# Jumpat/SegAnyGAussians

Hardware: AMD Instinct MI355X
Metric: train views/sec (fwd+bwd), 1080p, 1M Gaussians, 32-D features (higher is better)
Workload: dtype f32; 1 GPU; BASELINE cfg3: 1000000 Gaussians, 1920x1080, 32-D features, fwd+bwd, 1 view/GPU/step; parallelism=view-sharded x1

## Files before the change

### seganygaussians_amd/csrc/geometry.h

```cpp
#pragma once

#include "blend_rec.h"
#include "common.h"
#include "wave.h"

namespace mirast {

__device__ constexpr float SH_C0 = 0.28209479177387814f;
__device__ constexpr float SH_C1 = 0.4886025119029199f;
__device__ constexpr float SH_C2[5] = {1.0925484305920792f, -1.0925484305920792f, 0.31539156525252005f,
                                       -1.0925484305920792f, 0.5462742152960396f};
__device__ constexpr float SH_C3[7] = {-0.5900435899266435f, 2.890611442640554f, -0.4570457994644658f,
                                       0.3731763325901154f, -0.4570457994644658f, 1.445305721320277f,
                                       -0.5900435899266435f};

__device__ __forceinline__ void computeCov3D(const float3 scale, float mod, const float4 rot, float* cov3D)
{
    Mat3 S = {{{1.0f, 0, 0}, {0, 1.0f, 0}, {0, 0, 1.0f}}};
    S.m[0][0] = mod * scale.x;
    S.m[1][1] = mod * scale.y;
    S.m[2][2] = mod * scale.z;
    float r = rot.x, x = rot.y, y = rot.z, z = rot.w;
    Mat3 R = {{{1.f - 2.f * (y * y + z * z), 2.f * (x * y - r * z), 2.f * (x * z + r * y)},
               {2.f * (x * y + r * z), 1.f - 2.f * (x * x + z * z), 2.f * (y * z - r * x)},
// ... 311 lines not shown
    dL_dmean_acc.x += dm.x;
    dL_dmean_acc.y += dm.y;
    dL_dmean_acc.z += dm.z;
}

__device__ __forceinline__ void cov3d_backward(const float3 scale, float mod, const float4 rot, const float* dL_dcov3D,
                                               float3& dL_dscale, float4& dL_drot)
{
    const float r = rot.x, x = rot.y, y = rot.z, z = rot.w;
    const Mat3 R = {{{1.f - 2.f * (y * y + z * z), 2.f * (x * y - r * z), 2.f * (x * z + r * y)},
                     {2.f * (x * y + r * z), 1.f - 2.f * (x * x + z * z), 2.f * (y * z - r * x)},
                     {2.f * (x * z - r * y), 2.f * (y * z + r * x), 1.f - 2.f * (x * x + y * y)}}};
    Mat3 S = {{{1.0f, 0, 0}, {0, 1.0f, 0}, {0, 0, 1.0f}}};
    const float3 s = make_float3(mod * scale.x, mod * scale.y, mod * scale.z);
    S.m[0][0] = s.x;
    S.m[1][1] = s.y;
    S.m[2][2] = s.z;
    const Mat3 M = m3mul(S, R);
    const float* d = dL_dcov3D;
    const Mat3 dL_dSigma = {{{d[0], 0.5f * d[1], 0.5f * d[2]}, {0.5f * d[1], d[3], 0.5f * d[4]}, {0.5f * d[2], 0.5f * d[4], d[5]}}};
    Mat3 M2;
#pragma unroll
    for (int c = 0; c < 3; c++)
#pragma unroll
        for (int rr = 0; rr < 3; rr++) M2.m[c][rr] = 2.0f * M.m[c][rr];
    const Mat3 dL_dM = m3mul(M2, dL_dSigma);
    const Mat3 Rt = m3transpose(R);
    Mat3 dL_dMt = m3transpose(dL_dM);
    dL_dscale.x = Rt.m[0][0] * dL_dMt.m[0][0] + Rt.m[0][1] * dL_dMt.m[0][1] + Rt.m[0][2] * dL_dMt.m[0][2];
    dL_dscale.y = Rt.m[1][0] * dL_dMt.m[1][0] + Rt.m[1][1] * dL_dMt.m[1][1] + Rt.m[1][2] * dL_dMt.m[1][2];
    dL_dscale.z = Rt.m[2][0] * dL_dMt.m[2][0] + Rt.m[2][1] * dL_dMt.m[2][1] + Rt.m[2][2] * dL_dMt.m[2][2];
#pragma unroll
    for (int k = 0; k < 3; k++) {
        dL_dMt.m[0][k] *= s.x;
        dL_dMt.m[1][k] *= s.y;
        dL_dMt.m[2][k] *= s.z;
    }
    dL_drot.x = 2 * z * (dL_dMt.m[0][1] - dL_dMt.m[1][0]) + 2 * y * (dL_dMt.m[2][0] - dL_dMt.m[0][2]) + 2 * x * (dL_dMt.m[1][2] - dL_dMt.m[2][1]);
    dL_drot.y = 2 * y * (dL_dMt.m[1][0] + dL_dMt.m[0][1]) + 2 * z * (dL_dMt.m[2][0] + dL_dMt.m[0][2]) + 2 * r * (dL_dMt.m[1][2] - dL_dMt.m[2][1]) - 4 * x * (dL_dMt.m[2][2] + dL_dMt.m[1][1]);
    dL_drot.z = 2 * x * (dL_dMt.m[1][0] + dL_dMt.m[0][1]) + 2 * r * (dL_dMt.m[2][0] - dL_dMt.m[0][2]) + 2 * z * (dL_dMt.m[1][2] + dL_dMt.m[2][1]) - 4 * y * (dL_dMt.m[2][2] + dL_dMt.m[0][0]);
    dL_drot.w = 2 * r * (dL_dMt.m[0][1] - dL_dMt.m[1][0]) + 2 * x * (dL_dMt.m[2][0] + dL_dMt.m[0][2]) + 2 * y * (dL_dMt.m[1][2] + dL_dMt.m[2][1]) - 4 * z * (dL_dMt.m[1][1] + dL_dMt.m[0][0]);
}

__global__ void __launch_bounds__(256) geometry_bwd_kernel(
    int P, int D, int M, const float* __restrict__ means, const int* __restrict__ radii, const float* __restrict__ shs,
    const uint8_t* __restrict__ clamped, const float* __restrict__ scales, const float* __restrict__ rotations,
    const float* __restrict__ cov3Ds, ViewParams vp, const float* __restrict__ gpack ,
    float* __restrict__ dL_dmean2D, float* __restrict__ dL_dconics, float* __restrict__ dL_dopacity,
    float* __restrict__ dL_dmask, float* __restrict__ dL_dmeans, const float* __restrict__ dL_dcolor,
    float* __restrict__ dL_dcov, float* __restrict__ dL_dsh, float* __restrict__ dL_dscale, float* __restrict__ dL_drot)
{
    const int idx = blockIdx.x * blockDim.x + threadIdx.x;
    if (idx >= P) return;
    if (!(radii[idx] > 0)) {
        dL_dmean2D[3 * idx + 0] = dL_dmean2D[3 * idx + 1] = dL_dmean2D[3 * idx + 2] = 0.f;
        reinterpret_cast<float4*>(dL_dconics)[idx] = make_float4(0.f, 0.f, 0.f, 0.f);
        dL_dopacity[idx] = 0.f;
        if (dL_dmask) dL_dmask[idx] = 0.f;
#pragma unroll
        for (int i = 0; i < 6; i++) dL_dcov[(size_t)idx * 6 + i] = 0.f;
        dL_dmeans[3 * idx + 0] = dL_dmeans[3 * idx + 1] = dL_dmeans[3 * idx + 2] = 0.f;
        dL_dscale[3 * idx + 0] = dL_dscale[3 * idx + 1] = dL_dscale[3 * idx + 2] = 0.f;
        reinterpret_cast<float4*>(dL_drot)[idx] = make_float4(0.f, 0.f, 0.f, 0.f);
        return;
    }

    const float4 g0 = reinterpret_cast<const float4*>(gpack)[2 * idx];
    const float4 g1 = reinterpret_cast<const float4*>(gpack)[2 * idx + 1];
    dL_dmean2D[3 * idx + 0] = g0.x;
    dL_dmean2D[3 * idx + 1] = g0.y;
    dL_dmean2D[3 * idx + 2] = 0.f;
    reinterpret_cast<float4*>(dL_dconics)[idx] = make_float4(g0.z, g0.w, 0.f, g1.x);
    dL_dopacity[idx] = g1.y;
    if (dL_dmask) dL_dmask[idx] = g1.z;

    const float3 mean = make_float3(means[3 * idx], means[3 * idx + 1], means[3 * idx + 2]);
    const float3 dL_dconic = make_float3(g0.z, g0.w, g1.x);
    float cov3D[6];
#pragma unroll
    for (int i = 0; i < 6; i++) cov3D[i] = cov3Ds[(size_t)idx * 6 + i];
    Cov2DCtx c;
    cov2d_common(mean, vp, cov3D, c);
    const float h_x = vp.focal_x, h_y = vp.focal_y;
    const float limx = 1.3f * vp.tan_fovx;
    const float limy = 1.3f * vp.tan_fovy;
    const float x_grad_mul = c.txtz < -limx || c.txtz > limx ? 0 : 1;
    const float y_grad_mul = c.tytz < -limy || c.tytz > limy ? 0 : 1;
    const Mat3& T = c.T;
    const Mat3& Vrk = c.Vrk;
    const Mat3& Wm = c.W;
    const float3 t = c.t;
    const float a = c.cov.m[0][0];
    const float b = c.cov.m[0][1];
    const float cc = c.cov.m[1][1];
    const float denom = a * cc - b * b;
    float dL_da = 0, dL_db = 0, dL_dc = 0;
    const float denom2inv = 1.0f / ((denom * denom) + 0.0000001f);
    float dcov[6];
    if (denom2inv != 0) {
        dL_da = denom2inv * (-cc * cc * dL_dconic.x + 2 * b * cc * dL_dconic.y + (denom - a * cc) * dL_dconic.z);
        dL_dc = denom2inv * (-a * a * dL_dconic.z + 2 * a * b * dL_dconic.y + (denom - a * cc) * dL_dconic.x);
        dL_db = denom2inv * 2 * (b * cc * dL_dconic.x - (denom + 2 * b * b) * dL_dconic.y + a * b * dL_dconic.z);
        dcov[0] = (T.m[0][0] * T.m[0][0] * dL_da + T.m[0][0] * T.m[1][0] * dL_db + T.m[1][0] * T.m[1][0] * dL_dc);
        dcov[3] = (T.m[0][1] * T.m[0][1] * dL_da + T.m[0][1] * T.m[1][1] * dL_db + T.m[1][1] * T.m[1][1] * dL_dc);
        dcov[5] = (T.m[0][2] * T.m[0][2] * dL_da + T.m[0][2] * T.m[1][2] * dL_db + T.m[1][2] * T.m[1][2] * dL_dc);
        dcov[1] = 2 * T.m[0][0] * T.m[0][1] * dL_da + (T.m[0][0] * T.m[1][1] + T.m[0][1] * T.m[1][0]) * dL_db + 2 * T.m[1][0] * T.m[1][1] * dL_dc;
        dcov[2] = 2 * T.m[0][0] * T.m[0][2] * dL_da + (T.m[0][0] * T.m[1][2] + T.m[0][2] * T.m[1][0]) * dL_db + 2 * T.m[1][0] * T.m[1][2] * dL_dc;
        dcov[4] = 2 * T.m[0][2] * T.m[0][1] * dL_da + (T.m[0][1] * T.m[1][2] + T.m[0][2] * T.m[1][1]) * dL_db + 2 * T.m[1][1] * T.m[1][2] * dL_dc;
    } else {
#pragma unroll
        for (int i = 0; i < 6; i++) dcov[i] = 0;
    }
#pragma unroll
    for (int i = 0; i < 6; i++) dL_dcov[(size_t)idx * 6 + i] = dcov[i];

    const float dL_dT00 = 2 * (T.m[0][0] * Vrk.m[0][0] + T.m[0][1] * Vrk.m[0][1] + T.m[0][2] * Vrk.m[0][2]) * dL_da +
                          (T.m[1][0] * Vrk.m[0][0] + T.m[1][1] * Vrk.m[0][1] + T.m[1][2] * Vrk.m[0][2]) * dL_db;
    const float dL_dT01 = 2 * (T.m[0][0] * Vrk.m[1][0] + T.m[0][1] * Vrk.m[1][1] + T.m[0][2] * Vrk.m[1][2]) * dL_da +
                          (T.m[1][0] * Vrk.m[1][0] + T.m[1][1] * Vrk.m[1][1] + T.m[1][2] * Vrk.m[1][2]) * dL_db;
    const float dL_dT02 = 2 * (T.m[0][0] * Vrk.m[2][0] + T.m[0][1] * Vrk.m[2][1] + T.m[0][2] * Vrk.m[2][2]) * dL_da +
                          (T.m[1][0] * Vrk.m[2][0] + T.m[1][1] * Vrk.m[2][1] + T.m[1][2] * Vrk.m[2][2]) * dL_db;
    const float dL_dT10 = 2 * (T.m[1][0] * Vrk.m[0][0] + T.m[1][1] * Vrk.m[0][1] + T.m[1][2] * Vrk.m[0][2]) * dL_dc +
                          (T.m[0][0] * Vrk.m[0][0] + T.m[0][1] * Vrk.m[0][1] + T.m[0][2] * Vrk.m[0][2]) * dL_db;
    const float dL_dT11 = 2 * (T.m[1][0] * Vrk.m[1][0] + T.m[1][1] * Vrk.m[1][1] + T.m[1][2] * Vrk.m[1][2]) * dL_dc +
                          (T.m[0][0] * Vrk.m[1][0] + T.m[0][1] * Vrk.m[1][1] + T.m[0][2] * Vrk.m[1][2]) * dL_db;
    const float dL_dT12 = 2 * (T.m[1][0] * Vrk.m[2][0] + T.m[1][1] * Vrk.m[2][1] + T.m[1][2] * Vrk.m[2][2]) * dL_dc +
                          (T.m[0][0] * Vrk.m[2][0] + T.m[0][1] * Vrk.m[2][1] + T.m[0][2] * Vrk.m[2][2]) * dL_db;
    const float dL_dJ00 = Wm.m[0][0] * dL_dT00 + Wm.m[0][1] * dL_dT01 + Wm.m[0][2] * dL_dT02;
    const float dL_dJ02 = Wm.m[2][0] * dL_dT00 + Wm.m[2][1] * dL_dT01 + Wm.m[2][2] * dL_dT02;
    const float dL_dJ11 = Wm.m[1][0] * dL_dT10 + Wm.m[1][1] * dL_dT11 + Wm.m[1][2] * dL_dT12;
    const float dL_dJ12 = Wm.m[2][0] * dL_dT10 + Wm.m[2][1] * dL_dT11 + Wm.m[2][2] * dL_dT12;
    const float tz = 1.f / t.z;
    const float tz2 = tz * tz;
    const float tz3 = tz2 * tz;
    const float dL_dtx = x_grad_mul * -h_x * tz2 * dL_dJ02;
    const float dL_dty = y_grad_mul * -h_y * tz2 * dL_dJ12;
    const float dL_dtz = -h_x * tz2 * dL_dJ00 - h_y * tz2 * dL_dJ11 + (2 * h_x * t.x) * tz3 * dL_dJ02 + (2 * h_y * t.y) * tz3 * dL_dJ12;
    float3 dL_dmean_acc = transformVec4x3Transpose(make_float3(dL_dtx, dL_dty, dL_dtz), vp.view);

    const float* proj = vp.proj;
    const float4 m_hom = transformPoint4x4(mean, proj);
    const float m_w = 1.0f / (m_hom.w + 0.0000001f);
    const float mul1 = (proj[0] * mean.x + proj[4] * mean.y + proj[8] * mean.z + proj[12]) * m_w * m_w;
    const float mul2 = (proj[1] * mean.x + proj[5] * mean.y + proj[9] * mean.z + proj[13]) * m_w * m_w;
    const float gx = g0.x, gy = g0.y;
    float3 dm;
    dm.x = (proj[0] * m_w - proj[3] * mul1) * gx + (proj[1] * m_w - proj[3] * mul2) * gy;
    dm.y = (proj[4] * m_w - proj[7] * mul1) * gx + (proj[5] * m_w - proj[7] * mul2) * gy;
    dm.z = (proj[8] * m_w - proj[11] * mul1) * gx + (proj[9] * m_w - proj[11] * mul2) * gy;
    dL_dmean_acc.x += dm.x;
    dL_dmean_acc.y += dm.y;
    dL_dmean_acc.z += dm.z;
    if (shs) sh_backward(idx, D, M, mean, vp, shs, clamped, dL_dcolor, dL_dmean_acc, dL_dsh);
    dL_dmeans[3 * idx + 0] = dL_dmean_acc.x;
    dL_dmeans[3 * idx + 1] = dL_dmean_acc.y;
    dL_dmeans[3 * idx + 2] = dL_dmean_acc.z;
    if (scales) {
        const float3 s = make_float3(scales[3 * idx], scales[3 * idx + 1], scales[3 * idx + 2]);
        const float4 q = reinterpret_cast<const float4*>(rotations)[idx];
        float3 ds;
        float4 dq;
        cov3d_backward(s, vp.scale_modifier, q, dcov, ds, dq);
        dL_dscale[3 * idx + 0] = ds.x;
        dL_dscale[3 * idx + 1] = ds.y;
        dL_dscale[3 * idx + 2] = ds.z;
        reinterpret_cast<float4*>(dL_drot)[idx] = dq;
    } else {
        dL_dscale[3 * idx + 0] = dL_dscale[3 * idx + 1] = dL_dscale[3 * idx + 2] = 0.f;
        reinterpret_cast<float4*>(dL_drot)[idx] = make_float4(0.f, 0.f, 0.f, 0.f);
    }
}

__global__ void __launch_bounds__(256) unpack_mask_kernel(int P, const float* __restrict__ gpack, float* __restrict__ dL_dmask)
{
    const int idx = blockIdx.x * blockDim.x + threadIdx.x;
    if (idx < P) dL_dmask[idx] = gpack[(size_t)idx * 8 + 6];
}

}
```

### seganygaussians_amd/csrc/mi_rast.hip

```cpp
#include "host.h"

#include <algorithm>
#include <atomic>
#include <cstdio>
#include <cstdlib>
#include <cstring>
#include <mutex>
#include <type_traits>
#include <utility>
#include <vector>

#include "bin_full.h"
#include "bin_lean.h"
#include "tile_ranges.h"
#include "tile_sort.h"
#include "blend_bwd.h"
#include "blend_bwd_wave.h"
#include "blend_bwd_feat.h"
#include "blend_fwd.h"
#include "blend_fwd_wave.h"
#ifdef MI_RAST_PROFILING
#include "blend_fwd_x3.h"
#endif
#include "common.h"
// ... 406 lines not shown
                });
            }
        } else {
            hipLaunchKernelGGL(bin_spans_kernel<true>, dim3(bp.nwg), dim3(1024), span_lds_bytes((size_t)bp.lean_band_h * c.vp.grid_x), c.stream,
                               P, c.geom.index_rec, c.geom.depth_key, c.geom.band_bits, c.img.tile_count, c.img.tile_cursor, c.img.ranges, c.bin.entries,
                               c.vp.grid_x, c.vp.grid_y, bp.lean_band_h, bp.lean_nbands, (const int*)c.img.num_rendered, (int*)nullptr);
        }
    }
    STAGE_CHECK(c, "emit entries");
    if (verify) {
        uint32_t* ctr = reinterpret_cast<uint32_t*>(c.img.words() + NR_VERIFY);
        HIP_TRY(hipMemsetAsync(ctr, 0, sizeof(uint32_t), c.stream));
        hipLaunchKernelGGL(verify_entries_kernel, dim3(ntiles), dim3(256), 0, c.stream, (uint32_t)ntiles, c.img.ranges, c.bin.entries, ctr);
        uint32_t unwritten = 0;
        HIP_TRY(hipMemcpyAsync(&unwritten, ctr, sizeof(uint32_t), hipMemcpyDeviceToHost, c.stream));
        HIP_TRY(hipStreamSynchronize(c.stream));
        if (unwritten)
            return fail(MI_RAST_ERR_HIP, "internal error: " + std::to_string(unwritten) + " list slots were counted but not emitted "
                                         "(count / emit passes of bin_spans_kernel disagree)");
    }
    return MI_RAST_OK;
}

int take_longest_run(Call& c, const HostSync& hs, int dev)
{
    HIP_TRY(hipEventSynchronize(hs.ev2));
    c.longest_run = longest_of(hs.words() + NR_RUN_BOUNDS, c.ntiles());
    g_last_longest_run[dev] = (int)c.longest_run;
    return MI_RAST_OK;
}

template <int CLASS>
void launch_tile_sort_wave(const Call& c)
{
    hipLaunchKernelGGL(tile_sort_wave_kernel<CLASS>, dim3((c.ntiles() + 3) / 4), dim3(256), 0, c.stream, c.ntiles(), c.img.ranges,
                       (const uint2*)c.bin.entries, c.bin.blend_list);
}
template <int LO, int CAP, bool FB, int NT>
void launch_tile_sort(const Call& c)
{
    hipLaunchKernelGGL((tile_sort_kernel<LO, CAP, FB, NT>), dim3(c.ntiles()), dim3(NT), 0, c.stream, c.ntiles(), c.img.ranges, c.bin.entries,
                       c.bin.scratch, (const int*)(c.img.words() + NR_KEY_BITS), c.bin.blend_list);
}

int sort_stage(Call& c, const BinPlan& bp, const HostSync& hs, int dev, int R)
{
    {
        StageTimer t(c.stream, MI_STAGE_TILE_SORT);
        launch_tile_sort_wave<0>(c);
        if (int rc = take_longest_run(c, hs, dev)) return rc;
        if (bp.full ? hs.words()[NR_TOTAL] != R : hs.words()[NR_TOTAL] > R)
            return fail(MI_RAST_ERR_HIP, "internal error: tile counts do not add up to num_rendered");
        const int max_tile_count = hs.words()[NR_LONGEST];
        if (max_tile_count > 1024) launch_tile_sort_wave<1>(c);
        if (max_tile_count > 2048) launch_tile_sort_wave<2>(c);
        if (max_tile_count > TILE_SORT_WAVE_MAX) launch_tile_sort<TILE_SORT_WAVE_MAX, 6144, false, 1024>(c);
        if (max_tile_count > 6144) launch_tile_sort<6144, 8192, true, 1024>(c);
    }
    STAGE_CHECK(c, "tile sort");
    return MI_RAST_OK;
}

int geometry_and_binning(Call& c, const FrontArgs& a, int* num_rendered)
{
    const int dev = current_device();
    if (dev < 0) return fail(MI_RAST_ERR_HIP, "hipGetDevice failed (or device ordinal >= 64)");
    HostSync& hs = g_host_sync_tl[dev];
    BinPlan bp;
    if (int rc = plan_binning(c, bp)) return rc;
    size_t goff[MI_GEOM_NFIELDS], ioff[MI_IMG_NFIELDS], boff[MI_BIN_NFIELDS];
    char* geom_base = a.geometry_buffer(mi_rast_geometry_layout(c.P, goff), a.geometry_user);
    if (!geom_base) return fail(MI_RAST_ERR_ALLOC, "geometry buffer callback returned NULL");
    c.geom = geom_from(geom_base, c.P);
    char* img_base = a.image_buffer(mi_rast_image_layout(c.vp.W, c.vp.H, ioff), a.image_user);
    if (!img_base) return fail(MI_RAST_ERR_ALLOC, "image buffer callback returned NULL");
    c.img = img_from(img_base, c.vp.W, c.vp.H);

    if (int rc = preprocess_stage(c, a, bp)) return rc;
    if (int rc = opt_in_to_large_lds(dev)) return rc;
    if (!hs.init()) return fail(MI_RAST_ERR_HIP, "cannot allocate pinned host buffer / event");
    if (int rc = count_and_scan_stage(c, bp, hs)) return rc;
    HIP_TRY(hipEventRecord(hs.ev2, c.stream));
    HIP_TRY(hipEventSynchronize(hs.ev));
    long long Rsum = 0;
    for (int k = 0; k < R_SLOTS; k++) Rsum += hs.pinned[k * R_SLOT_STRIDE];
    if (Rsum > 0x7fffffffll) return fail(MI_RAST_ERR_INVALID, "more than 2^31 tile overlaps");
    const int R = (int)Rsum;
    *num_rendered = R;

    char* bin_base = a.binning_buffer(mi_rast_binning_layout(R, boff), a.binning_user);
    if (!bin_base) return fail(MI_RAST_ERR_ALLOC, "binning buffer callback returned NULL");
    c.bin = bin_from(bin_base, R);
    if (R == 0) return take_longest_run(c, hs, dev);
    if (int rc = emit_stage(c, bp, R)) return rc;
    return sort_stage(c, bp, hs, dev, R);
}

struct FwdArgs { int channels; const float *features, *mask, *bg; float *out_color, *out_mask, *out_depth; };
struct BwdArgs { int channels; const float *bg, *colors, *dL_dpix, *dL_dout_mask; float* dL_dcolor; };

template <int C, int EXTRA>
void launch_blend_fwd(const Call& c, const FwdArgs& a, ChannelBlock b)
{
    constexpr bool MAY_BE_PARTIAL = C == 16 && EXTRA == 0;
    with_bools(MAY_BE_PARTIAL && b.real < C, c.xexp(), [&](auto partial, auto xexp) {
        if constexpr (MAY_BE_PARTIAL || !decltype(partial)::value)
            hipLaunchKernelGGL((blend_fwd_kernel<C, EXTRA, decltype(xexp)::value, decltype(partial)::value>), dim3(c.vp.grid_x, c.vp.grid_y), dim3(256), 0,
                               c.stream, c.img.ranges, c.bin.blend_list, c.geom.index_rec, c.vp.W, c.vp.H, a.features + b.c0, a.mask, c.geom.depths,
// ... 522 lines not shown
```

### seganygaussians_amd/csrc/tile_sort.h

```cpp
#pragma once

#include "blend_rec.h"
#include "wave.h"

namespace mirast {

struct LdsPairs {
    uint32_t* k;
    uint32_t* v;
    __device__ __forceinline__ uint32_t key(int i) const { return k[i]; }
    __device__ __forceinline__ uint32_t val(int i) const { return v[i]; }
    __device__ __forceinline__ void set(int i, uint32_t kk, uint32_t vv) const
    {
        k[i] = kk;
        v[i] = vv;
    }
};
struct GlobalPairs {
    uint2* p;
    __device__ __forceinline__ uint32_t key(int i) const { return p[i].x; }
    __device__ __forceinline__ uint32_t val(int i) const { return p[i].y; }
    __device__ __forceinline__ void set(int i, uint32_t kk, uint32_t vv) const { p[i] = make_uint2(kk, vv); }
};

template <int NW, int MAXB, typename Src, typename Dst>
__device__ __forceinline__ void radix_pass(Src src, Dst dst, int n, int shift, uint32_t (*s_hist)[256], int tid)
{
    const int lane = tid & 63, wave = tid >> 6;
    const int chunks = (n + 63) >> 6;
    const int cpw = (chunks + NW - 1) / NW;
    const int begin = min(n, wave * cpw * 64), end = min(n, (wave + 1) * cpw * 64);
    for (int d = tid; d < NW * 256; d += NW * 64) (&s_hist[0][0])[d] = 0;
    __syncthreads();

    auto match = [&](uint32_t digit, bool active, uint32_t& rank_in_wave, uint32_t& cnt) {
        uint64_t m = ballot64(active);
#pragma unroll
        for (int b = 0; b < 8; b++) {
            const uint64_t bal = ballot64(active && ((digit >> b) & 1u));
            m &= ((digit >> b) & 1u) ? bal : ~bal;
        }
        rank_in_wave = __builtin_amdgcn_mbcnt_hi((uint32_t)(m >> 32), __builtin_amdgcn_mbcnt_lo((uint32_t)m, 0u));
        cnt = (uint32_t)__builtin_popcountll(m);
    };

    constexpr int NB = MAXB > 0 ? MAXB : 1;
    uint32_t c_key[NB], c_val[NB], c_rk[NB], c_cnt[NB];
    if (MAXB > 0) {
#pragma unroll
        for (int j = 0; j < NB; j++) {
            const int i0 = begin + 64 * j;
            if (i0 >= end) break;
            const int i = i0 + lane;
            const bool active = i < end;
            c_key[j] = active ? src.key(i) : 0u;
// ... 57 lines not shown
        for (int i0 = begin; i0 < end; i0 += 64) {
            const int i = i0 + lane;
            const bool active = i < end;
            const uint32_t key = active ? src.key(i) : 0u, val = active ? src.val(i) : 0u;
            uint32_t rk, cnt;
            match((key >> shift) & 0xFFu, active, rk, cnt);
            scatter(key, val, active, rk, cnt);
        }
    }
    __syncthreads();
}

template <int NW, typename Src>
__device__ __forceinline__ void emit_blend_list(Src sorted, int n, uint2 range, int tid, uint32_t* __restrict__ blend_list)
{
    uint32_t* out = blend_list + range.x;
    for (int i = tid; i < n; i += NW * 64) {
        const uint32_t k = sorted.key(i), v = sorted.val(i);
        int pos = i;
        if ((i > 0 && sorted.key(i - 1) == k) || (i + 1 < n && sorted.key(i + 1) == k)) {
            int lo = i, hi = i + 1;
            while (lo > 0 && sorted.key(lo - 1) == k) lo--;
            while (hi < n && sorted.key(hi) == k) hi++;
            int before = 0;
            for (int q = lo; q < hi; q++) before += (sorted.val(q) & ID_MASK) < (v & ID_MASK) ? 1 : 0;
            pos = lo + before;
        }
        out[pos] = v;
    }
}

__global__ void __launch_bounds__(256) verify_entries_kernel(uint32_t ntiles, const uint2* __restrict__ ranges,
                                                              const uint2* __restrict__ entries, uint32_t* __restrict__ unwritten)
{
    const uint32_t tile = blockIdx.x;
    if (tile >= ntiles) return;
    const uint2 r = ranges[tile];
    uint32_t n = 0;
    for (uint32_t i = r.x + threadIdx.x; i < r.y; i += 256) n += entries[i].y == 0u;
    if (n) atomicAdd(unwritten, n);
}

__device__ __forceinline__ void minmax64(double& lo, double& hi)
{
    double mn;
    asm("v_min_f64 %0, %1, %2" : "=v"(mn) : "v"(lo), "v"(hi));
    asm("v_max_f64 %0, %1, %2" : "=v"(hi) : "v"(lo), "v"(hi));
    lo = mn;
}

template <int EPL, int K, int J, bool FLIP>
__device__ __forceinline__ void bitonic_step(double (&a)[EPL], int lane)
{
    if constexpr (FLIP && K > EPL) {
        constexpr int M = K / EPL - 1;
        const bool lower = (lane & ((M + 1) >> 1)) == 0;
#pragma unroll
        for (int r = 0; r < EPL / 2; r++) {
            double x0 = a[r], y0 = lane_xor64<M>(a[EPL - 1 - r]);
            double x1 = a[EPL - 1 - r], y1 = lane_xor64<M>(a[r]);
            minmax64(x0, y0);
            minmax64(x1, y1);
            a[r] = lower ? x0 : y0;
            a[EPL - 1 - r] = lower ? x1 : y1;
        }
    } else if constexpr (!FLIP && J >= EPL) {
        constexpr int M = J / EPL;
        const bool lower = (lane & M) == 0;
#pragma unroll
        for (int r = 0; r < EPL; r++) {
            double x = a[r], y = lane_xor64<M>(a[r]);
            minmax64(x, y);
            a[r] = lower ? x : y;
        }
    } else {
        constexpr int X = FLIP ? K - 1 : J;
#pragma unroll
        for (int r = 0; r < EPL; r++)
            if ((r ^ X) > r) minmax64(a[r], a[r ^ X]);
    }
}
template <int EPL, int K, int J>
__device__ __forceinline__ void bitonic_tail(double (&a)[EPL], int lane)
{
    if constexpr (J >= 1) {
        bitonic_step<EPL, K, J, false>(a, lane);
        bitonic_tail<EPL, K, J / 2>(a, lane);
    } else if constexpr (K < 64 * EPL) {
        bitonic_step<EPL, 2 * K, 0, true>(a, lane);
        bitonic_tail<EPL, 2 * K, K / 2>(a, lane);
    }
}

template <int EPL>
__device__ __forceinline__ void tile_sort_in_wave(const uint2* __restrict__ seg, int n, uint32_t* __restrict__ out, int lane)
{
    double a[EPL];
#pragma unroll
    for (int r = 0; r < EPL; r++) {
        const int e = r * 64 + lane;
        uint64_t w = 0x7FEFFFFFFFFFFFFFull;
        if (e < n) {
            const uint2 p = seg[e];
            w = ((uint64_t)p.x << 32) | __builtin_rotateleft32(p.y, 4);
        }
        a[r] = __builtin_bit_cast(double, w);
    }
    bitonic_step<EPL, 2, 0, true>(a, lane);
    bitonic_tail<EPL, 2, 0>(a, lane);
#pragma unroll
    for (int r = 0; r < EPL; r++) {
        const int e = lane * EPL + r;
        if (e < n) out[e] = __builtin_rotateright32((uint32_t)__builtin_bit_cast(uint64_t, a[r]), 4);
    }
}

constexpr int TILE_SORT_WAVE_MAX = 4096;
template <int CLASS>
__global__ void __launch_bounds__(256) tile_sort_wave_kernel(uint32_t ntiles, const uint2* __restrict__ ranges,
                                                              const uint2* __restrict__ entries, uint32_t* __restrict__ blend_list)
{
    const int lane = threadIdx.x & 63;
    const uint32_t tile = blockIdx.x * 4u + (threadIdx.x >> 6);
    if (tile >= ntiles) return;
    const uint2 range = ranges[tile];
    const int n = (int)(range.y - range.x);
    const uint2* seg = entries + range.x;
    uint32_t* out = blend_list + range.x;
    if constexpr (CLASS == 2) {
        if (n > 2048 && n <= 4096) tile_sort_in_wave<64>(seg, n, out, lane);
    } else if constexpr (CLASS == 1) {
        if (n > 1024 && n <= 2048) tile_sort_in_wave<32>(seg, n, out, lane);
    } else {
        if (n == 0 || n > 1024) return;
        if (n <= 256) tile_sort_in_wave<4>(seg, n, out, lane);
        else if (n <= 512) tile_sort_in_wave<8>(seg, n, out, lane);
        else tile_sort_in_wave<16>(seg, n, out, lane);
    }
}

template <int LO, int CAP, bool GLOBAL_FALLBACK, int NT>
__global__ void __launch_bounds__(NT) tile_sort_kernel(uint32_t ntiles, const uint2* __restrict__ ranges,
                                                        uint2* __restrict__ entries, uint2* __restrict__ scratch,
                                                        const int* __restrict__ key_bits, uint32_t* __restrict__ blend_list)
{
    __shared__ uint32_t s_k[2][CAP];
    __shared__ uint32_t s_v[2][CAP];
    constexpr int NW = NT / 64;
    __shared__ uint32_t s_hist[NW][256];
    const int tid = threadIdx.x;
    const uint32_t tile = blockIdx.x;
    if (tile >= ntiles) return;
    const uint2 range = ranges[tile];
    const int passes = (*key_bits + 7) >> 3;
    const int n = (int)(range.y - range.x);
    if (n <= LO) return;
    if (n > CAP && !GLOBAL_FALLBACK) return;
    uint2* seg = entries + range.x;
    if (n <= CAP) {
        for (int i = tid; i < n; i += NT) {
            const uint2 e = seg[i];
            s_k[0][i] = e.x;
            s_v[0][i] = e.y;
        }
        __syncthreads();
        int cur = 0;
        for (int p = 0; p < passes; p++, cur ^= 1)
            radix_pass<NW, (CAP + NW * 64 - 1) / (NW * 64)>(LdsPairs{s_k[cur], s_v[cur]}, LdsPairs{s_k[cur ^ 1], s_v[cur ^ 1]}, n, 8 * p, s_hist, tid);
        emit_blend_list<NW>(LdsPairs{s_k[cur], s_v[cur]}, n, range, tid, blend_list);
    } else {
        uint2* a = seg;
        uint2* b = scratch + range.x;
        for (int p = 0; p < passes; p++) {
            radix_pass<NW, 0>(GlobalPairs{a}, GlobalPairs{b}, n, 8 * p, s_hist, tid);
            uint2* t = a;
            a = b;
            b = t;
        }
        emit_blend_list<NW>(GlobalPairs{a}, n, range, tid, blend_list);
    }
}

}
```

Measured before the change: 910.5 views/s.

## Add 3/4-size in-wave sort classes and skip zero-gradient rows in geometry backward

Adds an in-lane sorting network that handles element-per-lane counts of 6, 12, 24 and 48, and splits the tile-sort size classes so tiles of 257-384, 513-768, 1025-1536 and 2049-3072 entries are padded less. It also restructures the geometry backward kernel to skip the full gradient computation when all packed 2D gradients are zero and no SH or mask gradients are needed, writing zeros from a single store path. The new sorting network and extra kernel launch add code complexity and a compile-time risk for non-power-of-two bitonic correctness.

Result: no change. 914.9 views/s, median of 6 (+0.5%).

```diff
diff --git a/seganygaussians_amd/csrc/geometry.h b/seganygaussians_amd/csrc/geometry.h
--- a/seganygaussians_amd/csrc/geometry.h
+++ b/seganygaussians_amd/csrc/geometry.h
@@ -387,123 +387,113 @@
 {
     const int idx = blockIdx.x * blockDim.x + threadIdx.x;
     if (idx >= P) return;
-    if (!(radii[idx] > 0)) {
-        dL_dmean2D[3 * idx + 0] = dL_dmean2D[3 * idx + 1] = dL_dmean2D[3 * idx + 2] = 0.f;
-        reinterpret_cast<float4*>(dL_dconics)[idx] = make_float4(0.f, 0.f, 0.f, 0.f);
-        dL_dopacity[idx] = 0.f;
-        if (dL_dmask) dL_dmask[idx] = 0.f;
-#pragma unroll
-        for (int i = 0; i < 6; i++) dL_dcov[(size_t)idx * 6 + i] = 0.f;
-        dL_dmeans[3 * idx + 0] = dL_dmeans[3 * idx + 1] = dL_dmeans[3 * idx + 2] = 0.f;
-        dL_dscale[3 * idx + 0] = dL_dscale[3 * idx + 1] = dL_dscale[3 * idx + 2] = 0.f;
-        reinterpret_cast<float4*>(dL_drot)[idx] = make_float4(0.f, 0.f, 0.f, 0.f);
-        return;
-    }
-
-    const float4 g0 = reinterpret_cast<const float4*>(gpack)[2 * idx];
-    const float4 g1 = reinterpret_cast<const float4*>(gpack)[2 * idx + 1];
+    bool zero_row = !(radii[idx] > 0);
+    float4 g0 = make_float4(0.f, 0.f, 0.f, 0.f), g1 = g0;
+    if (!zero_row) {
+        g0 = reinterpret_cast<const float4*>(gpack)[2 * idx];
+        g1 = reinterpret_cast<const float4*>(gpack)[2 * idx + 1];
+        zero_row = shs == nullptr && dL_dmask == nullptr && g0.x == 0.f && g0.y == 0.f && g0.z == 0.f && g0.w == 0.f && g1.x == 0.f &&
+                   g1.y == 0.f;
+    }
+    float dcov[6] = {0.f, 0.f, 0.f, 0.f, 0.f, 0.f};
+    float3 dmean = make_float3(0.f, 0.f, 0.f), ds = make_float3(0.f, 0.f, 0.f);
+    float4 dq = make_float4(0.f, 0.f, 0.f, 0.f);
+    if (!zero_row) {
+        const float3 mean = make_float3(means[3 * idx], means[3 * idx + 1], means[3 * idx + 2]);
+        const float3 dL_dconic = make_float3(g0.z, g0.w, g1.x);
+        float cov3D[6];
+#pragma unroll
+        for (int i = 0; i < 6; i++) cov3D[i] = cov3Ds[(size_t)idx * 6 + i];
+        Cov2DCtx c;
+        cov2d_common(mean, vp, cov3D, c);
+        const float h_x = vp.focal_x, h_y = vp.focal_y;
+        const float limx = 1.3f * vp.tan_fovx;
+        const float limy = 1.3f * vp.tan_fovy;
+        const float x_grad_mul = c.txtz < -limx || c.txtz > limx ? 0 : 1;
+        const float y_grad_mul = c.tytz < -limy || c.tytz > limy ? 0 : 1;
+        const Mat3& T = c.T;
+        const Mat3& Vrk = c.Vrk;
+        const Mat3& Wm = c.W;
+        const float3 t = c.t;
+        const float a = c.cov.m[0][0];
+        const float b = c.cov.m[0][1];
+        const float cc = c.cov.m[1][1];
+        const float denom = a * cc - b * b;
+        float dL_da = 0, dL_db = 0, dL_dc = 0;
+        const float denom2inv = 1.0f / ((denom * denom) + 0.0000001f);
+        if (denom2inv != 0) {
+            dL_da = denom2inv * (-cc * cc * dL_dconic.x + 2 * b * cc * dL_dconic.y + (denom - a * cc) * dL_dconic.z);
+            dL_dc = denom2inv * (-a * a * dL_dconic.z + 2 * a * b * dL_dconic.y + (denom - a * cc) * dL_dconic.x);
+            dL_db = denom2inv * 2 * (b * cc * dL_dconic.x - (denom + 2 * b * b) * dL_dconic.y + a * b * dL_dconic.z);
+            dcov[0] = (T.m[0][0] * T.m[0][0] * dL_da + T.m[0][0] * T.m[1][0] * dL_db + T.m[1][0] * T.m[1][0] * dL_dc);
+            dcov[3] = (T.m[0][1] * T.m[0][1] * dL_da + T.m[0][1] * T.m[1][1] * dL_db + T.m[1][1] * T.m[1][1] * dL_dc);
+            dcov[5] = (T.m[0][2] * T.m[0][2] * dL_da + T.m[0][2] * T.m[1][2] * dL_db + T.m[1][2] * T.m[1][2] * dL_dc);
+            dcov[1] = 2 * T.m[0][0] * T.m[0][1] * dL_da + (T.m[0][0] * T.m[1][1] + T.m[0][1] * T.m[1][0]) * dL_db + 2 * T.m[1][0] * T.m[1][1] * dL_dc;
+            dcov[2] = 2 * T.m[0][0] * T.m[0][2] * dL_da + (T.m[0][0] * T.m[1][2] + T.m[0][2] * T.m[1][0]) * dL_db + 2 * T.m[1][0] * T.m[1][2] * dL_dc;
+            dcov[4] = 2 * T.m[0][2] * T.m[0][1] * dL_da + (T.m[0][1] * T.m[1][2] + T.m[0][2] * T.m[1][1]) * dL_db + 2 * T.m[1][1] * T.m[1][2] * dL_dc;
+        }
+
+        const float dL_dT00 = 2 * (T.m[0][0] * Vrk.m[0][0] + T.m[0][1] * Vrk.m[0][1] + T.m[0][2] * Vrk.m[0][2]) * dL_da +
+                              (T.m[1][0] * Vrk.m[0][0] + T.m[1][1] * Vrk.m[0][1] + T.m[1][2] * Vrk.m[0][2]) * dL_db;
+        const float dL_dT01 = 2 * (T.m[0][0] * Vrk.m[1][0] + T.m[0][1] * Vrk.m[1][1] + T.m[0][2] * Vrk.m[1][2]) * dL_da +
+                              (T.m[1][0] * Vrk.m[1][0] + T.m[1][1] * Vrk.m[1][1] + T.m[1][2] * Vrk.m[1][2]) * dL_db;
+        const float dL_dT02 = 2 * (T.m[0][0] * Vrk.m[2][0] + T.m[0][1] * Vrk.m[2][1] + T.m[0][2] * Vrk.m[2][2]) * dL_da +
+                              (T.m[1][0] * Vrk.m[2][0] + T.m[1][1] * Vrk.m[2][1] + T.m[1][2] * Vrk.m[2][2]) * dL_db;
+        const float dL_dT10 = 2 * (T.m[1][0] * Vrk.m[0][0] + T.m[1][1] * Vrk.m[0][1] + T.m[1][2] * Vrk.m[0][2]) * dL_dc +
+                              (T.m[0][0] * Vrk.m[0][0] + T.m[0][1] * Vrk.m[0][1] + T.m[0][2] * Vrk.m[0][2]) * dL_db;
+        const float dL_dT11 = 2 * (T.m[1][0] * Vrk.m[1][0] + T.m[1][1] * Vrk.m[1][1] + T.m[1][2] * Vrk.m[1][2]) * dL_dc +
+                              (T.m[0][0] * Vrk.m[1][0] + T.m[0][1] * Vrk.m[1][1] + T.m[0][2] * Vrk.m[1][2]) * dL_db;
+        const float dL_dT12 = 2 * (T.m[1][0] * Vrk.m[2][0] + T.m[1][1] * Vrk.m[2][1] + T.m[1][2] * Vrk.m[2][2]) * dL_dc +
+                              (T.m[0][0] * Vrk.m[2][0] + T.m[0][1] * Vrk.m[2][1] + T.m[0][2] * Vrk.m[2][2]) * dL_db;
+        const float dL_dJ00 = Wm.m[0][0] * dL_dT00 + Wm.m[0][1] * dL_dT01 + Wm.m[0][2] * dL_dT02;
+        const float dL_dJ02 = Wm.m[2][0] * dL_dT00 + Wm.m[2][1] * dL_dT01 + Wm.m[2][2] * dL_dT02;
+        const float dL_dJ11 = Wm.m[1][0] * dL_dT10 + Wm.m[1][1] * dL_dT11 + Wm.m[1][2] * dL_dT12;
+        const float dL_dJ12 = Wm.m[2][0] * dL_dT10 + Wm.m[2][1] * dL_dT11 + Wm.m[2][2] * dL_dT12;
+        const float tz = 1.f / t.z;
+        const float tz2 = tz * tz;
+        const float tz3 = tz2 * tz;
+        const float dL_dtx = x_grad_mul * -h_x * tz2 * dL_dJ02;
+        const float dL_dty = y_grad_mul * -h_y * tz2 * dL_dJ12;
+        const float dL_dtz = -h_x * tz2 * dL_dJ00 - h_y * tz2 * dL_dJ11 + (2 * h_x * t.x) * tz3 * dL_dJ02 + (2 * h_y * t.y) * tz3 * dL_dJ12;
+        float3 dL_dmean_acc = transformVec4x3Transpose(make_float3(dL_dtx, dL_dty, dL_dtz), vp.view);
+
+        const float* proj = vp.proj;
+        const float4 m_hom = transformPoint4x4(mean, proj);
+        const float m_w = 1.0f / (m_hom.w + 0.0000001f);
+        const float mul1 = (proj[0] * mean.x + proj[4] * mean.y + proj[8] * mean.z + proj[12]) * m_w * m_w;
+        const float mul2 = (proj[1] * mean.x + proj[5] * mean.y + proj[9] * mean.z + proj[13]) * m_w * m_w;
+        const float gx = g0.x, gy = g0.y;
+        float3 dm;
+        dm.x = (proj[0] * m_w - proj[3] * mul1) * gx + (proj[1] * m_w - proj[3] * mul2) * gy;
+        dm.y = (proj[4] * m_w - proj[7] * mul1) * gx + (proj[5] * m_w - proj[7] * mul2) * gy;
+        dm.z = (proj[8] * m_w - proj[11] * mul1) * gx + (proj[9] * m_w - proj[11] * mul2) * gy;
+        dL_dmean_acc.x += dm.x;
+        dL_dmean_acc.y += dm.y;
+        dL_dmean_acc.z += dm.z;
+        if (shs) sh_backward(idx, D, M, mean, vp, shs, clamped, dL_dcolor, dL_dmean_acc, dL_dsh);
+        dmean = dL_dmean_acc;
+        if (scales) {
+            const float3 s = make_float3(scales[3 * idx], scales[3 * idx + 1], scales[3 * idx + 2]);
+            const float4 q = reinterpret_cast<const float4*>(rotations)[idx];
+            cov3d_backward(s, vp.scale_modifier, q, dcov, ds, dq);
+        }
+    }
+
     dL_dmean2D[3 * idx + 0] = g0.x;
     dL_dmean2D[3 * idx + 1] = g0.y;
     dL_dmean2D[3 * idx + 2] = 0.f;
     reinterpret_cast<float4*>(dL_dconics)[idx] = make_float4(g0.z, g0.w, 0.f, g1.x);
     dL_dopacity[idx] = g1.y;
     if (dL_dmask) dL_dmask[idx] = g1.z;
-
-    const float3 mean = make_float3(means[3 * idx], means[3 * idx + 1], means[3 * idx + 2]);
-    const float3 dL_dconic = make_float3(g0.z, g0.w, g1.x);
-    float cov3D[6];
-#pragma unroll
-    for (int i = 0; i < 6; i++) cov3D[i] = cov3Ds[(size_t)idx * 6 + i];
-    Cov2DCtx c;
-    cov2d_common(mean, vp, cov3D, c);
-    const float h_x = vp.focal_x, h_y = vp.focal_y;
-    const float limx = 1.3f * vp.tan_fovx;
-    const float limy = 1.3f * vp.tan_fovy;
-    const float x_grad_mul = c.txtz < -limx || c.txtz > limx ? 0 : 1;
-    const float y_grad_mul = c.tytz < -limy || c.tytz > limy ? 0 : 1;
-    const Mat3& T = c.T;
-    const Mat3& Vrk = c.Vrk;
-    const Mat3& Wm = c.W;
-    const float3 t = c.t;
-    const float a = c.cov.m[0][0];
-    const float b = c.cov.m[0][1];
-    const float cc = c.cov.m[1][1];
-    const float denom = a * cc - b * b;
-    float dL_da = 0, dL_db = 0, dL_dc = 0;
-    const float denom2inv = 1.0f / ((denom * denom) + 0.0000001f);
-    float dcov[6];
-    if (denom2inv != 0) {
-        dL_da = denom2inv * (-cc * cc * dL_dconic.x + 2 * b * cc * dL_dconic.y + (denom - a * cc) * dL_dconic.z);
-        dL_dc = denom2inv * (-a * a * dL_dconic.z + 2 * a * b * dL_dconic.y + (denom - a * cc) * dL_dconic.x);
-        dL_db = denom2inv * 2 * (b * cc * dL_dconic.x - (denom + 2 * b * b) * dL_dconic.y + a * b * dL_dconic.z);
-        dcov[0] = (T.m[0][0] * T.m[0][0] * dL_da + T.m[0][0] * T.m[1][0] * dL_db + T.m[1][0] * T.m[1][0] * dL_dc);
-        dcov[3] = (T.m[0][1] * T.m[0][1] * dL_da + T.m[0][1] * T.m[1][1] * dL_db + T.m[1][1] * T.m[1][1] * dL_dc);
-        dcov[5] = (T.m[0][2] * T.m[0][2] * dL_da + T.m[0][2] * T.m[1][2] * dL_db + T.m[1][2] * T.m[1][2] * dL_dc);
-        dcov[1] = 2 * T.m[0][0] * T.m[0][1] * dL_da + (T.m[0][0] * T.m[1][1] + T.m[0][1] * T.m[1][0]) * dL_db + 2 * T.m[1][0] * T.m[1][1] * dL_dc;
-        dcov[2] = 2 * T.m[0][0] * T.m[0][2] * dL_da + (T.m[0][0] * T.m[1][2] + T.m[0][2] * T.m[1][0]) * dL_db + 2 * T.m[1][0] * T.m[1][2] * dL_dc;
-        dcov[4] = 2 * T.m[0][2] * T.m[0][1] * dL_da + (T.m[0][1] * T.m[1][2] + T.m[0][2] * T.m[1][1]) * dL_db + 2 * T.m[1][1] * T.m[1][2] * dL_dc;
-    } else {
-#pragma unroll
-        for (int i = 0; i < 6; i++) dcov[i] = 0;
-    }
 #pragma unroll
     for (int i = 0; i < 6; i++) dL_dcov[(size_t)idx * 6 + i] = dcov[i];
-
-    const float dL_dT00 = 2 * (T.m[0][0] * Vrk.m[0][0] + T.m[0][1] * Vrk.m[0][1] + T.m[0][2] * Vrk.m[0][2]) * dL_da +
-                          (T.m[1][0] * Vrk.m[0][0] + T.m[1][1] * Vrk.m[0][1] + T.m[1][2] * Vrk.m[0][2]) * dL_db;
-    const float dL_dT01 = 2 * (T.m[0][0] * Vrk.m[1][0] + T.m[0][1] * Vrk.m[1][1] + T.m[0][2] * Vrk.m[1][2]) * dL_da +
-                          (T.m[1][0] * Vrk.m[1][0] + T.m[1][1] * Vrk.m[1][1] + T.m[1][2] * Vrk.m[1][2]) * dL_db;
-    const float dL_dT02 = 2 * (T.m[0][0] * Vrk.m[2][0] + T.m[0][1] * Vrk.m[2][1] + T.m[0][2] * Vrk.m[2][2]) * dL_da +
-                          (T.m[1][0] * Vrk.m[2][0] + T.m[1][1] * Vrk.m[2][1] + T.m[1][2] * Vrk.m[2][2]) * dL_db;
-    const float dL_dT10 = 2 * (T.m[1][0] * Vrk.m[0][0] + T.m[1][1] * Vrk.m[0][1] + T.m[1][2] * Vrk.m[0][2]) * dL_dc +
-                          (T.m[0][0] * Vrk.m[0][0] + T.m[0][1] * Vrk.m[0][1] + T.m[0][2] * Vrk.m[0][2]) * dL_db;
-    const float dL_dT11 = 2 * (T.m[1][0] * Vrk.m[1][0] + T.m[1][1] * Vrk.m[1][1] + T.m[1][2] * Vrk.m[1][2]) * dL_dc +
-                          (T.m[0][0] * Vrk.m[1][0] + T.m[0][1] * Vrk.m[1][1] + T.m[0][2] * Vrk.m[1][2]) * dL_db;
-    const float dL_dT12 = 2 * (T.m[1][0] * Vrk.m[2][0] + T.m[1][1] * Vrk.m[2][1] + T.m[1][2] * Vrk.m[2][2]) * dL_dc +
-                          (T.m[0][0] * Vrk.m[2][0] + T.m[0][1] * Vrk.m[2][1] + T.m[0][2] * Vrk.m[2][2]) * dL_db;
-    const float dL_dJ00 = Wm.m[0][0] * dL_dT00 + Wm.m[0][1] * dL_dT01 + Wm.m[0][2] * dL_dT02;
-    const float dL_dJ02 = Wm.m[2][0] * dL_dT00 + Wm.m[2][1] * dL_dT01 + Wm.m[2][2] * dL_dT02;
-    const float dL_dJ11 = Wm.m[1][0] * dL_dT10 + Wm.m[1][1] * dL_dT11 + Wm.m[1][2] * dL_dT12;
-    const float dL_dJ12 = Wm.m[2][0] * dL_dT10 + Wm.m[2][1] * dL_dT11 + Wm.m[2][2] * dL_dT12;
-    const float tz = 1.f / t.z;
-    const float tz2 = tz * tz;
-    const float tz3 = tz2 * tz;
-    const float dL_dtx = x_grad_mul * -h_x * tz2 * dL_dJ02;
-    const float dL_dty = y_grad_mul * -h_y * tz2 * dL_dJ12;
-    const float dL_dtz = -h_x * tz2 * dL_dJ00 - h_y * tz2 * dL_dJ11 + (2 * h_x * t.x) * tz3 * dL_dJ02 + (2 * h_y * t.y) * tz3 * dL_dJ12;
-    float3 dL_dmean_acc = transformVec4x3Transpose(make_float3(dL_dtx, dL_dty, dL_dtz), vp.view);
-
-    const float* proj = vp.proj;
-    const float4 m_hom = transformPoint4x4(mean, proj);
-    const float m_w = 1.0f / (m_hom.w + 0.0000001f);
-    const float mul1 = (proj[0] * mean.x + proj[4] * mean.y + proj[8] * mean.z + proj[12]) * m_w * m_w;
-    const float mul2 = (proj[1] * mean.x + proj[5] * mean.y + proj[9] * mean.z + proj[13]) * m_w * m_w;
-    const float gx = g0.x, gy = g0.y;
-    float3 dm;
-    dm.x = (proj[0] * m_w - proj[3] * mul1) * gx + (proj[1] * m_w - proj[3] * mul2) * gy;
-    dm.y = (proj[4] * m_w - proj[7] * mul1) * gx + (proj[5] * m_w - proj[7] * mul2) * gy;
-    dm.z = (proj[8] * m_w - proj[11] * mul1) * gx + (proj[9] * m_w - proj[11] * mul2) * gy;
-    dL_dmean_acc.x += dm.x;
-    dL_dmean_acc.y += dm.y;
-    dL_dmean_acc.z += dm.z;
-    if (shs) sh_backward(idx, D, M, mean, vp, shs, clamped, dL_dcolor, dL_dmean_acc, dL_dsh);
-    dL_dmeans[3 * idx + 0] = dL_dmean_acc.x;
-    dL_dmeans[3 * idx + 1] = dL_dmean_acc.y;
-    dL_dmeans[3 * idx + 2] = dL_dmean_acc.z;
-    if (scales) {
-        const float3 s = make_float3(scales[3 * idx], scales[3 * idx + 1], scales[3 * idx + 2]);
-        const float4 q = reinterpret_cast<const float4*>(rotations)[idx];
-        float3 ds;
-        float4 dq;
-        cov3d_backward(s, vp.scale_modifier, q, dcov, ds, dq);
-        dL_dscale[3 * idx + 0] = ds.x;
-        dL_dscale[3 * idx + 1] = ds.y;
-        dL_dscale[3 * idx + 2] = ds.z;
-        reinterpret_cast<float4*>(dL_drot)[idx] = dq;
-    } else {
-        dL_dscale[3 * idx + 0] = dL_dscale[3 * idx + 1] = dL_dscale[3 * idx + 2] = 0.f;
-        reinterpret_cast<float4*>(dL_drot)[idx] = make_float4(0.f, 0.f, 0.f, 0.f);
-    }
+    dL_dmeans[3 * idx + 0] = dmean.x;
+    dL_dmeans[3 * idx + 1] = dmean.y;
+    dL_dmeans[3 * idx + 2] = dmean.z;
+    dL_dscale[3 * idx + 0] = ds.x;
+    dL_dscale[3 * idx + 1] = ds.y;
+    dL_dscale[3 * idx + 2] = ds.z;
+    reinterpret_cast<float4*>(dL_drot)[idx] = dq;
 }
 
 __global__ void __launch_bounds__(256) unpack_mask_kernel(int P, const float* __restrict__ gpack, float* __restrict__ dL_dmask)
diff --git a/seganygaussians_amd/csrc/mi_rast.hip b/seganygaussians_amd/csrc/mi_rast.hip
--- a/seganygaussians_amd/csrc/mi_rast.hip
+++ b/seganygaussians_amd/csrc/mi_rast.hip
@@ -482,8 +482,9 @@
         if (bp.full ? hs.words()[NR_TOTAL] != R : hs.words()[NR_TOTAL] > R)
             return fail(MI_RAST_ERR_HIP, "internal error: tile counts do not add up to num_rendered");
         const int max_tile_count = hs.words()[NR_LONGEST];
-        if (max_tile_count > 1024) launch_tile_sort_wave<1>(c);
-        if (max_tile_count > 2048) launch_tile_sort_wave<2>(c);
+        if (max_tile_count > tile_sort_class_lo(1)) launch_tile_sort_wave<1>(c);
+        if (max_tile_count > tile_sort_class_lo(2)) launch_tile_sort_wave<2>(c);
+        if (max_tile_count > tile_sort_class_lo(3)) launch_tile_sort_wave<3>(c);
         if (max_tile_count > TILE_SORT_WAVE_MAX) launch_tile_sort<TILE_SORT_WAVE_MAX, 6144, false, 1024>(c);
         if (max_tile_count > 6144) launch_tile_sort<6144, 8192, true, 1024>(c);
     }
diff --git a/seganygaussians_amd/csrc/sort_network.h b/seganygaussians_amd/csrc/sort_network.h
--- /dev/null
+++ b/seganygaussians_amd/csrc/sort_network.h
@@ -0,0 +1,75 @@
+#pragma once
+
+#if defined(__HIPCC__)
+#define MI_SORTNET_FN __host__ __device__ inline __attribute__((always_inline))
+#else
+#define MI_SORTNET_FN inline __attribute__((always_inline))
+#endif
+
+namespace mirast {
+
+constexpr bool three_quarter(int epl) { return (epl & (epl - 1)) != 0; }
+
+constexpr int in_lane_partner(int r, int K, int J, bool flip)
+{
+    if (flip) {
+        const int p = r / K * K + (K - 1 - r % K);
+        return p > r ? p : -1;
+    }
+    return (r / J) % 2 == 0 ? r + J : -1;
+}
+
+template <int EPL, int K, int J, bool FLIP, typename T, typename CE>
+MI_SORTNET_FN void in_lane_step(T (&a)[EPL], CE ce)
+{
+    if constexpr (!FLIP && J == 1 && three_quarter(EPL)) {
+#pragma unroll
+        for (int r = 0; r < EPL; r += 3) {
+            ce(a[r], a[r + 2]);
+            ce(a[r], a[r + 1]);
+            ce(a[r + 1], a[r + 2]);
+        }
+    } else {
+#pragma unroll
+        for (int r = 0; r < EPL; r++) {
+            const int p = in_lane_partner(r, K, J, FLIP);
+            if (p >= 0) ce(a[r], a[p]);
+        }
+    }
+}
+
+template <int EPL, int J, typename T, typename CE>
+MI_SORTNET_FN void in_lane_tail(T (&a)[EPL], CE ce)
+{
+    if constexpr (J >= 1) {
+        in_lane_step<EPL, 0, J, false>(a, ce);
+        in_lane_tail<EPL, J / 2>(a, ce);
+    }
+}
+template <int EPL, typename T, typename CE>
+MI_SORTNET_FN void in_lane_merge(T (&a)[EPL], CE ce)
+{
+    in_lane_tail<EPL, EPL / 2>(a, ce);
+}
+
+template <int EPL, int K, typename T, typename CE>
+MI_SORTNET_FN void in_lane_stages(T (&a)[EPL], CE ce)
+{
+    if constexpr (K <= EPL) {
+        in_lane_step<EPL, K, 0, true>(a, ce);
+        in_lane_tail<EPL, K / 4>(a, ce);
+        in_lane_stages<EPL, 2 * K>(a, ce);
+    }
+}
+template <int EPL, typename T, typename CE>
+MI_SORTNET_FN void in_lane_sort(T (&a)[EPL], CE ce)
+{
+    if constexpr (three_quarter(EPL)) {
+        in_lane_step<EPL, 3, 1, false>(a, ce);
+        in_lane_stages<EPL, 6>(a, ce);
+    } else {
+        in_lane_stages<EPL, 2>(a, ce);
+    }
+}
+
+}
diff --git a/seganygaussians_amd/csrc/tile_sort.h b/seganygaussians_amd/csrc/tile_sort.h
--- a/seganygaussians_amd/csrc/tile_sort.h
+++ b/seganygaussians_amd/csrc/tile_sort.h
@@ -1,6 +1,7 @@
 #pragma once
 
 #include "blend_rec.h"
+#include "sort_network.h"
 #include "wave.h"
 
 namespace mirast {
@@ -164,7 +165,7 @@
 template <int EPL, int K, int J, bool FLIP>
 __device__ __forceinline__ void bitonic_step(double (&a)[EPL], int lane)
 {
-    if constexpr (FLIP && K > EPL) {
+    if constexpr (FLIP) {
         constexpr int M = K / EPL - 1;
         const bool lower = (lane & ((M + 1) >> 1)) == 0;
 #pragma unroll
@@ -176,7 +177,7 @@
             a[r] = lower ? x0 : y0;
             a[EPL - 1 - r] = lower ? x1 : y1;
         }
-    } else if constexpr (!FLIP && J >= EPL) {
+    } else {
         constexpr int M = J / EPL;
         const bool lower = (lane & M) == 0;
 #pragma unroll
@@ -185,22 +186,20 @@
             minmax64(x, y);
             a[r] = lower ? x : y;
         }
-    } else {
-        constexpr int X = FLIP ? K - 1 : J;
-#pragma unroll
-        for (int r = 0; r < EPL; r++)
-            if ((r ^ X) > r) minmax64(a[r], a[r ^ X]);
     }
 }
 template <int EPL, int K, int J>
 __device__ __forceinline__ void bitonic_tail(double (&a)[EPL], int lane)
 {
-    if constexpr (J >= 1) {
+    if constexpr (J >= EPL) {
         bitonic_step<EPL, K, J, false>(a, lane);
         bitonic_tail<EPL, K, J / 2>(a, lane);
-    } else if constexpr (K < 64 * EPL) {
-        bitonic_step<EPL, 2 * K, 0, true>(a, lane);
-        bitonic_tail<EPL, 2 * K, K / 2>(a, lane);
+    } else {
+        in_lane_merge(a, [](double& lo, double& hi) { minmax64(lo, hi); });
+        if constexpr (K < 64 * EPL) {
+            bitonic_step<EPL, 2 * K, 0, true>(a, lane);
+            bitonic_tail<EPL, 2 * K, K / 2>(a, lane);
+        }
     }
 }
 
@@ -218,8 +217,9 @@
         }
         a[r] = __builtin_bit_cast(double, w);
     }
-    bitonic_step<EPL, 2, 0, true>(a, lane);
-    bitonic_tail<EPL, 2, 0>(a, lane);
+    in_lane_sort(a, [](double& lo, double& hi) { minmax64(lo, hi); });
+    bitonic_step<EPL, 2 * EPL, 0, true>(a, lane);
+    bitonic_tail<EPL, 2 * EPL, EPL / 2>(a, lane);
 #pragma unroll
     for (int r = 0; r < EPL; r++) {
         const int e = lane * EPL + r;
@@ -228,6 +228,8 @@
 }
 
 constexpr int TILE_SORT_WAVE_MAX = 4096;
+constexpr int tile_sort_class_lo(int cls) { return cls == 0 ? 0 : cls == 1 ? 1024 : cls == 2 ? 2048 : 3072; }
+constexpr int tile_sort_class_hi(int cls) { return cls == 0 ? 1024 : cls == 1 ? 2048 : cls == 2 ? 3072 : 4096; }
 template <int CLASS>
 __global__ void __launch_bounds__(256) tile_sort_wave_kernel(uint32_t ntiles, const uint2* __restrict__ ranges,
                                                               const uint2* __restrict__ entries, uint32_t* __restrict__ blend_list)
@@ -239,14 +241,19 @@
     const int n = (int)(range.y - range.x);
     const uint2* seg = entries + range.x;
     uint32_t* out = blend_list + range.x;
-    if constexpr (CLASS == 2) {
-        if (n > 2048 && n <= 4096) tile_sort_in_wave<64>(seg, n, out, lane);
+    if (n <= tile_sort_class_lo(CLASS) || n > tile_sort_class_hi(CLASS)) return;
+    if constexpr (CLASS == 3) {
+        tile_sort_in_wave<64>(seg, n, out, lane);
+    } else if constexpr (CLASS == 2) {
+        tile_sort_in_wave<48>(seg, n, out, lane);
     } else if constexpr (CLASS == 1) {
-        if (n > 1024 && n <= 2048) tile_sort_in_wave<32>(seg, n, out, lane);
-    } else {
-        if (n == 0 || n > 1024) return;
+        if (n <= 1536) tile_sort_in_wave<24>(seg, n, out, lane);
+        else tile_sort_in_wave<32>(seg, n, out, lane);
+    } else {
         if (n <= 256) tile_sort_in_wave<4>(seg, n, out, lane);
+        else if (n <= 384) tile_sort_in_wave<6>(seg, n, out, lane);
         else if (n <= 512) tile_sort_in_wave<8>(seg, n, out, lane);
+        else if (n <= 768) tile_sort_in_wave<12>(seg, n, out, lane);
         else tile_sort_in_wave<16>(seg, n, out, lane);
     }
 }
```
